# lauradarcy/gym-craftingworld

Measured on AMD Instinct MI355X. Metric: env-steps/sec at 65536 envs, 1/2/4/8 MI355X; bit-exact vs CPU ref, higher is better.
Workload: dtype u8

## Files before the change

### gym_craftingworld_amd/csrc/cw_kernels.hip

```cpp
#include <hip/hip_runtime.h>
#include <stdint.h>

#include "cw_host.h"
#include "cw_layout.h"
#include "cw_mt.h"

#define CW_WAVE 64
#define CW_BALLOT(p) __builtin_amdgcn_ballot_w64(p)
#define CW_ALT_FRAME_PACE 2

#ifdef CW_TRACE
__device__ unsigned long long cw_trace_buf[1024 * 8];
#define CW_STAMP(env, k) do { if (lane == 0) { cw_trace_buf[((env) & 1023) * 8 + (k)] = wall_clock64(); \
                                               if ((k) == 0 || (k) == 5) cw_trace_buf[((env) & 1023) * 8 + 6 + ((k) ? 1 : 0)] = clock64(); } } while (0)
extern "C" hipError_t cwk_trace_read(unsigned long long *dst) { return hipMemcpyFromSymbol(dst, HIP_SYMBOL(cw_trace_buf), sizeof(cw_trace_buf)); }
#else
#define CW_STAMP(env, k) do { } while (0)
#endif

enum { EMPTY = 0, STICKS = 1, AXE = 2, HAMMER = 3, ROCK = 4, TREE = 5, BREAD = 6, HOUSE = 7, WHEAT = 8 };
enum { T_MAKEBREAD = 0, T_EATBREAD = 1, T_BUILDHOUSE = 2, T_CHOPTREE = 3, T_CHOPROCK = 4,
       T_GOTOHOUSE = 5, T_MOVEAXE = 6, T_MOVEHAMMER = 7, T_MOVESTICKS = 8 };

typedef uint32_t u32x3 __attribute__((ext_vector_type(3)));
typedef u32x3 u32x3_a4 __attribute__((aligned(4)));

__device__ __forceinline__ void unpack_pos(const uint4 &v, uint32_t sp[8])
{
    sp[0] = v.x & 0xFFFFu; sp[1] = v.x >> 16;
    sp[2] = v.y & 0xFFFFu; sp[3] = v.y >> 16;
    sp[4] = v.z & 0xFFFFu; sp[5] = v.z >> 16;
    sp[6] = v.w & 0xFFFFu; sp[7] = v.w >> 16;
}
__device__ __forceinline__ uint4 pack_pos(const uint32_t sp[8])
{
    return make_uint4(sp[0] | (sp[1] << 16), sp[2] | (sp[3] << 16), sp[4] | (sp[5] << 16), sp[6] | (sp[7] << 16));
}
__device__ __forceinline__ int slot_at(const uint32_t sp[8], uint32_t cell)
{
    int idx = -1;
#pragma unroll
    for (int k = 0; k < 8; k++) idx = (sp[k] == cell) ? k : idx;
    return idx;
}
__device__ __forceinline__ uint32_t code_of(uint32_t codes, int idx)
{
    return idx < 0 ? 0u : ((codes >> (4 * idx)) & 15u);
}
__device__ __forceinline__ uint32_t rgb_of_code(uint32_t code)
{
    uint32_t c = 0;
    c = code == 1 ? (110u | (69u << 8) | (39u << 16)) : c;
    c = code == 2 ? (255u | (105u << 8) | (180u << 16)) : c;
    c = code == 3 ? (100u | (100u << 8) | (200u << 16)) : c;
    c = code == 4 ? (100u | (100u << 8) | (100u << 16)) : c;
    c = code == 5 ? (0u | (128u << 8) | (0u << 16)) : c;
    c = code == 6 ? (205u | (133u << 8) | (63u << 16)) : c;
    c = code == 7 ? (197u | (91u << 8) | (97u << 16)) : c;
    c = code == 8 ? (240u | (230u << 8) | (140u << 16)) : c;
    return c;
}

__device__ __forceinline__ u32x3 cell_row_dwords(uint32_t rgb)
{
    u32x3 d;
    d.x = rgb | (rgb << 24);
    d.y = (rgb >> 8) | (rgb << 16);
    d.z = (rgb >> 16) | (rgb << 8);
    return d;
}
__device__ __forceinline__ u32x3 overlay_dwords(u32x3 d, uint32_t o)
{
    d.x = (d.x & 0x00FFFFFFu) | (o << 24);
    d.y = (o >> 8) | (o << 16);
    d.z = (d.z & 0xFFFFFF00u) | (o >> 16);
    return d;
}
__device__ __forceinline__ u32x3 onehot_dwords(uint32_t bits)
{
    u32x3 d;
    d.x = (bits & 1u) | ((bits >> 1 & 1u) << 8) | ((bits >> 2 & 1u) << 16) | ((bits >> 3 & 1u) << 24);
    d.y = (bits >> 4 & 1u) | ((bits >> 5 & 1u) << 8) | ((bits >> 6 & 1u) << 16) | ((bits >> 7 & 1u) << 24);
    d.z = (bits >> 8 & 1u) | ((bits >> 9 & 1u) << 8) | ((bits >> 10 & 1u) << 16) | ((bits >> 11 & 1u) << 24);
    return d;
}

__device__ __forceinline__ void paint_cell(uint8_t *frame, int S, uint32_t cell, uint32_t code,
                                           bool agent_here, uint32_t hold, uint32_t div_magic, bool mark_rows_only = false)
{
    const uint32_t r = __umulhi(cell, div_magic);
    const uint32_t c = cell - r * S;
    const uint32_t rgb = rgb_of_code(code);
    const u32x3 base = cell_row_dwords(rgb);
    const uint32_t row_bytes = 12u * S;
    uint8_t *p = frame + (size_t)(4u * r) * row_bytes + 12u * c;
#pragma unroll
    for (int dy = 0; dy < 4; dy++) {
        u32x3 d = base;
        if (agent_here && (dy == 1 || dy == 2)) {
            uint32_t o = (dy == 2 && hold != 0) ? rgb_of_code(hold) : 0x00FFFFFFu;
            d = overlay_dwords(d, o);
        }
        if (dy == 1 || dy == 2 || !mark_rows_only) *(u32x3_a4 *)(p + dy * row_bytes) = d;
    }
}

__device__ __forceinline__ uint32_t cpv_color(int k)
{
    return k == 0 ? (45u | (82u << 8) | (160u << 16)) : k == 1 ? (255u | (102u << 8) | (102u << 16))
         : k == 2 ? (204u | (204u << 8)) : k == 3 ? (211u | (211u << 8) | (211u << 16))
         : k == 4 ? (34u | (133u << 8) | (34u << 16)) : k == 5 ? ((215u << 8) | (255u << 16))
         : k == 6 ? (153u | (52u << 8) | (255u << 16)) : k == 7 ? (10u | (215u << 8) | (100u << 16)) : (255u << 16);
}
__device__ __forceinline__ void alt_paint_tile(uint8_t *frame, int S, uint32_t r, uint32_t c, uint32_t code,
                                               bool agent_here, uint32_t hold)
{
    const uint32_t row_bytes = 9u * S;
    uint8_t *p = frame + (size_t)(3u * r) * row_bytes + 9u * c;
#pragma unroll
    for (int k = 0; k < 9; k++) {
        uint32_t cnt = (k < 8) ? (code == (uint32_t)(k + 1) ? 1u : 0u) : (agent_here ? 1u : 0u);
        if (k < 3) cnt += (agent_here && hold == (uint32_t)(k + 1)) ? 1u : 0u;
        const uint32_t col = cpv_color(k);
        uint8_t *q = p + (k / 3) * row_bytes + (k % 3) * 3;
        q[0] = (uint8_t)(cnt * (col & 0xFFu));
        q[1] = (uint8_t)(cnt * ((col >> 8) & 0xFFu));
        q[2] = (uint8_t)(cnt * ((col >> 16) & 0xFFu));
    }
}
__device__ __forceinline__ void alt_paint_strip(uint8_t *frame, int S, uint32_t hold, uint32_t first, uint32_t step,
                                                bool whole)
// ... 55 lines not shown
            for (int z = 0; z < pace; z++) __builtin_amdgcn_s_sleep(1);
        }
        if (p_any) {
            dst[p_off] = (uint8_t)p_val;
            dst[p_off + 1] = (uint8_t)(p_val >> 8);
            dst[p_off + 2] = (uint8_t)(p_val >> 16);
        }
    }
}

__device__ __forceinline__ void render_frame(uint8_t *__restrict__ dst0, uint8_t *__restrict__ dst1,
                                             int S, int ncell, uint32_t div_magic, const uint32_t sp[8],
                                             const uint32_t rgb[8], uint32_t agent_cell, uint32_t hold_rgb,
                                             int lane)
{
    const uint32_t row_bytes = 12u * S;
    for (uint32_t cell = lane; cell < (uint32_t)ncell; cell += CW_WAVE) {
        const uint32_t r = __umulhi(cell, div_magic);
        const uint32_t c = cell - r * S;
        uint32_t col = 0;
#pragma unroll
        for (int k = 0; k < 8; k++) col = (cell == sp[k]) ? rgb[k] : col;
        const u32x3 d = cell_row_dwords(col);
        const bool ag = (cell == agent_cell);
        const u32x3 d1 = ag ? overlay_dwords(d, 0x00FFFFFFu) : d;
        const u32x3 d2 = ag ? overlay_dwords(d, hold_rgb) : d;
        const size_t off = (size_t)(4u * r) * row_bytes + 12u * c;
        uint8_t *q = dst0 + off;
        *(u32x3_a4 *)(q) = d;
        *(u32x3_a4 *)(q + row_bytes) = d1;
        *(u32x3_a4 *)(q + 2 * row_bytes) = d2;
        *(u32x3_a4 *)(q + 3 * row_bytes) = d;
        if (dst1) {
            uint8_t *q1 = dst1 + off;
            *(u32x3_a4 *)(q1) = d;
            *(u32x3_a4 *)(q1 + row_bytes) = d1;
            *(u32x3_a4 *)(q1 + 2 * row_bytes) = d2;
            *(u32x3_a4 *)(q1 + 3 * row_bytes) = d;
        }
    }
}
template <bool kRecords = false>
__device__ __forceinline__ void paint_state_frame(const CwParams &P, uint8_t *dst, const uint32_t sp[8], uint32_t codes, uint32_t agent_cell,
                                                  uint32_t hold, int lane, uint8_t *dst1 = nullptr)
{
    if (P.raster == 1) {
        render_frame_alt<kRecords>(dst, dst1, P.size, P.ncell, P.div_magic, sp, codes, agent_cell, hold, lane, CW_ALT_FRAME_PACE);
    } else {
        uint32_t rgb[8];
#pragma unroll
        for (int k = 0; k < 8; k++) rgb[k] = rgb_of_code((codes >> (4 * k)) & 15u);
        render_frame(dst, dst1, P.size, P.ncell, P.div_magic, sp, rgb, agent_cell, hold ? rgb_of_code(hold) : 0x00FFFFFFu, lane);
    }
}
__device__ __forceinline__ uint32_t agent_cell_of(const CwParams &P, uint32_t hx) { return (hx & 0xFFu) * P.size + ((hx >> 8) & 0xFFu); }
__device__ __forceinline__ uint32_t hold_of(uint32_t hx) { return (hx >> 16) & 0xFFu; }
enum { CW_SRC_CURRENT = 0, CW_SRC_INIT = 1, CW_SRC_GOAL = 2 };
__device__ __forceinline__ void load_state_uniform(const CwParams &P, int env, int src, uint32_t sp[8], uint32_t &codes, uint32_t &agent_cell, uint32_t &hold)
{
    uint4 v_p;
    uint32_t v_c, v_a, v_h = 0;
    if (src == CW_SRC_CURRENT) {
        const uint4 h = P.hdr[env];
        v_p = P.pos[env];
        v_c = h.w;
        v_a = agent_cell_of(P, h.x);
        v_h = hold_of(h.x);
    } else if (src == CW_SRC_INIT) {
        v_p = P.init_pos[env];
        v_c = CW_CODES_INITIAL;
        v_a = P.init_agent[env];
    } else {
        v_p = P.goal_pos[env];
        v_c = P.goal_codes[env];
        v_a = P.goal_agent[env];
    }
    unpack_pos(make_uint4(__builtin_amdgcn_readfirstlane(v_p.x), __builtin_amdgcn_readfirstlane(v_p.y), __builtin_amdgcn_readfirstlane(v_p.z),
                          __builtin_amdgcn_readfirstlane(v_p.w)), sp);
    codes = __builtin_amdgcn_readfirstlane(v_c);
    agent_cell = __builtin_amdgcn_readfirstlane(v_a);
    hold = __builtin_amdgcn_readfirstlane(v_h);
}

struct CwStepOut {
    int reward;
    bool done, success, invalid, changed;
    uint32_t dirty0, dirty1;
    bool mark0, mark1;
    uint32_t step_num, achieved, desired;
    uint32_t n_success;
};

__device__ __forceinline__ int32_t episode_return_of(const CwParams &P, const CwStepOut &o)
{
    return (int32_t)o.n_success * (P.max_steps + 1) - (int32_t)o.step_num;
}

template <typename InitPosFn>
__device__ __forceinline__ CwStepOut step_env(const CwParams &P, uint4 &h, uint32_t sp[8], int a, InitPosFn load_init_pos)
{
    CwStepOut o;
    const int S = P.size;
    int ar = h.x & 0xFF, ac = (h.x >> 8) & 0xFF;
    uint32_t hold = (h.x >> 16) & 0xFF;
    uint32_t achieved = h.y & 0xFFFFu;
    const uint32_t desired = h.y >> 16;
    const uint32_t step_num = min((h.z & 0xFFFFu) + 1u, 0xFFFFu);
    const uint32_t flags = (h.z >> 16) & ~CW_FLAG_RESET;
    uint32_t codes = h.w;

    o.invalid = (unsigned)a > 5u;
    bool changed = false;
    const uint32_t cell = ar * S + ac;
    const int idx_here = slot_at(sp, cell);
    const uint32_t code_here = code_of(codes, idx_here);
    o.dirty0 = cell;
    o.dirty1 = 0xFFFFFFFFu;
    o.mark0 = o.mark1 = false;

    if (a == 4) {
        if (code_here >= STICKS && code_here <= HAMMER && hold == 0) {
            hold = code_here;
#pragma unroll
            for (int k = 0; k < 8; k++) sp[k] = (k == idx_here) ? CW_POS_HELD : sp[k];
            changed = true;
        }
    } else if (a == 5) {
        if (hold != 0 && idx_here < 0) {
#pragma unroll
            for (int k = 0; k < 8; k++) sp[k] = (sp[k] == CW_POS_HELD) ? cell : sp[k];
            hold = 0;
            changed = true;
        }
    } else if (!o.invalid) {
        const int dr = (a == 0) ? -1 : (a == 2) ? 1 : 0;
        const int dc = (a == 1) ? 1 : (a == 3) ? -1 : 0;
        const int nr = min(max(ar + dr, 0), S - 1);
        const int nc = min(max(ac + dc, 0), S - 1);
        uint32_t old_obj = 0;
        uint32_t cur_code = code_here;
        if (nr != ar || nc != ac) {
            const uint32_t ncell = nr * S + nc;
            const int idx_t = slot_at(sp, ncell);
            const uint32_t t = code_of(codes, idx_t);
            const bool cant = (t == ROCK && hold != 3) || (t == TREE && hold != 2);
            if (!cant) {
                changed = true;
                o.dirty1 = ncell;
                o.mark0 = true;
                ar = nr; ac = nc;
                old_obj = t;
                uint32_t nw = t;
                if (t == ROCK || t == BREAD) nw = EMPTY;
                else if (t == TREE) nw = STICKS;
                else if (t == STICKS && hold == 3) nw = HOUSE;
                else if (t == WHEAT && hold == 2) nw = BREAD;
                if (nw != t) {
                    codes = (codes & ~(15u << (4 * idx_t))) | (nw << (4 * idx_t));
                    if (nw == EMPTY) {
#pragma unroll
                        for (int k = 0; k < 8; k++) sp[k] = (k == idx_t) ? CW_POS_GONE : sp[k];
                    }
                }
                cur_code = nw;
                o.mark1 = nw == t;
            }
        }
        const uint32_t pcell = ar * S + ac;
        if (old_obj == BREAD) achieved |= 1u << T_EATBREAD;
        else if (old_obj == ROCK) achieved |= 1u << T_CHOPROCK;
        else if (old_obj == TREE) achieved |= 1u << T_CHOPTREE;
        achieved = (cur_code == HOUSE) ? (achieved | (1u << T_GOTOHOUSE))
                                       : (achieved & ~(1u << T_GOTOHOUSE));
        if (hold != 0) {
            const uint4 ip = load_init_pos();
            const uint32_t ip_sticks = ip.x & 0xFFFFu, ip_axe = ip.x >> 16;
            const uint32_t ip_hammer = ip.y & 0xFFFFu, ip_tree = ip.z & 0xFFFFu;
            if (hold == 1) {
                const bool home = (pcell == ip_sticks) ||
                                  (pcell == ip_tree && (achieved & (1u << T_CHOPTREE)));
                achieved = home ? (achieved & ~(1u << T_MOVESTICKS)) : (achieved | (1u << T_MOVESTICKS));
            } else if (hold == 2) {
                if (old_obj == WHEAT) achieved |= 1u << T_MAKEBREAD;
                achieved = (pcell == ip_axe) ? (achieved & ~(1u << T_MOVEAXE)) : (achieved | (1u << T_MOVEAXE));
            } else {
                if (old_obj == STICKS) achieved |= 1u << T_BUILDHOUSE;
                achieved = (pcell == ip_hammer) ? (achieved & ~(1u << T_MOVEHAMMER)) : (achieved | (1u << T_MOVEHAMMER));
            }
        }
    }

    int reward = -1;
    if (changed) {
        const uint32_t am = achieved & P.task_mask, dm = desired & P.task_mask;
        bool hit;
        if (flags & CW_FLAG_SUBSET)
            hit = ((dm & ~am) == 0) && (((~(dm ^ am)) & P.task_mask) != 0);
        else
            hit = (am == dm);
        reward = hit ? P.max_steps : -1;
    }
    o.reward = reward;
    o.changed = changed;
    o.success = (reward == P.max_steps);
    o.done = (step_num >= (uint32_t)P.max_steps) || o.success;
    o.step_num = step_num;
    o.achieved = achieved;
    o.desired = desired;
    o.n_success = min((flags >> 2) + (o.success ? 1u : 0u), 0x3FFFu);

    h.x = (uint32_t)ar | ((uint32_t)ac << 8) | (hold << 16) | (h.x & 0xFF000000u);
    h.y = achieved | (desired << 16);
    h.z = step_num | (((flags & 3u) | (o.n_success << 2)) << 16);
    h.w = codes;
    return o;
}

__device__ __forceinline__ void paint_changed_cells(const CwParams &P, int env, const uint4 &h, const uint32_t sp[8], const CwStepOut &o)
{
    uint8_t *frame = P.obs + (size_t)env * P.frame_bytes;
    const uint32_t hold = hold_of(h.x);
    const uint32_t acell = agent_cell_of(P, h.x);
    if (P.raster == 1) {
        const uint32_t r0 = __umulhi(o.dirty0, P.div_magic);
        alt_paint_tile(frame, P.size, r0, o.dirty0 - r0 * P.size, code_of(h.w, slot_at(sp, o.dirty0)), o.dirty0 == acell, hold);
        if (o.dirty1 != 0xFFFFFFFFu) {
            const uint32_t r1 = __umulhi(o.dirty1, P.div_magic);
            alt_paint_tile(frame, P.size, r1, o.dirty1 - r1 * P.size, code_of(h.w, slot_at(sp, o.dirty1)), o.dirty1 == acell, hold);
        }
        alt_paint_strip(frame, P.size, hold, 0, 1, false);
    } else {
        paint_cell(frame, P.size, o.dirty0, code_of(h.w, slot_at(sp, o.dirty0)), o.dirty0 == acell, hold, P.div_magic, o.mark0);
        if (o.dirty1 != 0xFFFFFFFFu)
            paint_cell(frame, P.size, o.dirty1, code_of(h.w, slot_at(sp, o.dirty1)), o.dirty1 == acell, hold, P.div_magic, o.mark1);
    }
}

__device__ __forceinline__ void store_step_outputs(const CwParams &P, int env, const CwStepOut &o)
{
    P.reward[env] = o.reward;
    P.done[env] = o.done ? 1 : 0;
    P.achieved_out[env] = (uint16_t)o.achieved;
    P.desired_out[env] = (uint16_t)o.desired;
    if (o.done) { P.episode_length[env] = (int32_t)o.step_num; P.episode_return[env] = episode_return_of(P, o); }
}

__device__ __forceinline__ int load_action(const void *actions, int act_dtype, int i)
{
    if (act_dtype == 0) return ((const int32_t *)actions)[i];
    if (act_dtype == 1) { const long long a = ((const long long *)actions)[i]; return a == (long long)(int)a ? (int)a : -1; }
    return ((const uint8_t *)actions)[i];
}

struct CwGoalState { uint4 pos; uint32_t codes, agent; };
__device__ __forceinline__ bool pop_next_episode(const CwParams &P, int env, uint32_t ctl, uint4 &h, uint32_t sp[8], bool count_episode, CwGoalState *goal = nullptr)
{
    const uint32_t slot = ctl & 0xFFu;
    const size_t at = (size_t)slot * P.n_envs + env;
    const uint4 m = P.nx_misc[at];
    const uint4 ipos = P.nx_init_pos[at];
    const uint4 gpos = P.nx_goal_pos[at];
    const int32_t ep_no = count_episode ? P.ep_no[env] : 0;
    if (!(m.z >> 31)) return false;
    P.init_pos[env] = ipos;
    P.goal_pos[env] = gpos;
    if (goal) { goal->pos = gpos; goal->codes = m.y; goal->agent = m.x >> 16; }
    P.goal_codes[env] = m.y;
    P.init_agent[env] = (uint16_t)(m.x & 0xFFFFu);
    P.goal_agent[env] = (uint16_t)(m.x >> 16);
    if (count_episode) P.ep_no[env] = ep_no + 1;
    ((uint32_t *)(P.nx_misc + at))[2] = 0;
    P.nx_ctl[env] = (slot + 1u == CW_LA_DEPTH ? 0u : slot + 1u) | CW_CTL_QUEUED;
    const uint32_t ia = m.x & 0xFFFFu;
    const uint32_t ar = __umulhi(ia, P.div_magic), ac = ia - ar * P.size;
    h.x = ar | (ac << 8) | (h.x & 0xFF000000u);
    h.y = (m.z & 0xFFFFu) << 16;
    h.z = (CW_FLAG_RESET | (((m.z >> 16) & 1u) ? CW_FLAG_SUBSET : 0u)) << 16;
    h.w = CW_CODES_INITIAL;
    unpack_pos(ipos, sp);
    return true;
}

__device__ __forceinline__ void note_slow_reset(const CwParams &P, int env, uint32_t ctl)
{
    atomicAdd(&P.counters[5], 1ull);
    if (!(ctl & CW_CTL_QUEUED)) P.nx_ctl[env] = ctl | CW_CTL_QUEUED;
}

__global__ __launch_bounds__(256) void cw_step_kernel(CwParams P, const void *actions, int act_dtype, int paint_dirty)
{
    const int i = blockIdx.x * blockDim.x + threadIdx.x;
    if (i == 0) {
        atomicAdd(&P.counters[0], (unsigned long long)P.n_envs);
    }
    const bool live = i < P.n_envs;
    bool done = false, success = false, invalid = false;
    if (live) {
        const int a = load_action(actions, act_dtype, i);
        uint4 h = P.hdr[i];
        uint32_t sp[8];
        unpack_pos(P.pos[i], sp);
        const CwStepOut o = step_env(P, h, sp, a, [&]() { return P.init_pos[i]; });
        done = o.done; success = o.success; invalid = o.invalid;

        P.hdr[i] = h;
        P.pos[i] = pack_pos(sp);
        store_step_outputs(P, i, o);
        if (paint_dirty && o.changed) paint_changed_cells(P, i, h, sp, o);
    }
    const unsigned long long m_done = CW_BALLOT(done), m_succ = CW_BALLOT(success), m_inv = CW_BALLOT(invalid);
    if ((m_done | m_inv) && (threadIdx.x & (CW_WAVE - 1)) == 0) {
        if (m_done) atomicAdd(&P.counters[1], (unsigned long long)__popcll(m_done));
        if (m_succ) atomicAdd(&P.counters[2], (unsigned long long)__popcll(m_succ));
        if (m_inv) atomicAdd(&P.counters[3], (unsigned long long)__popcll(m_inv));
    }
}

template <int A>
__device__ __forceinline__ void expand_one(const CwParams &P, const uint4 *__restrict__ hdr_in, const uint4 *__restrict__ pos_in, int j, int env, size_t row,
                                           const CwExpandOut &O)
{
    uint4 h = hdr_in[j];
    uint32_t sp[8];
    unpack_pos(pos_in[j], sp);
    const CwStepOut o = step_env(P, h, sp, A, [&]() { return P.init_pos[env]; });
    if (O.reward) O.reward[row] = o.reward;
    if (O.done) O.done[row] = o.done ? 1 : 0;
    if (O.changed) O.changed[row] = o.changed ? 1 : 0;
    if (O.achieved) O.achieved[row] = (uint16_t)o.achieved;
    if (O.hdr) O.hdr[row] = h;
    if (O.pos) O.pos[row] = pack_pos(sp);
}

__global__ __launch_bounds__(256) void cw_expand_kernel(CwParams P, const int32_t *__restrict__ env_of, const uint4 *__restrict__ hdr_in,
                                                        const uint4 *__restrict__ pos_in, int n_states, CwExpandOut O)
{
    const int j = (int)(blockIdx.x * blockDim.x + threadIdx.x);
    const int a = (int)blockIdx.y;
    int env = -1;
    bool skipped = false;
    if (j < n_states) {
        if (env_of) {
            const int32_t v = env_of[j];
            if (cwh_expand_env_ok(v, P.n_envs)) env = v;
            else skipped = v >= 0;
        } else {
            env = j < P.n_envs ? j : (int)((uint32_t)j % (uint32_t)P.n_envs);
        }
    }
    if (a == 0) {
        const unsigned long long m_skip = CW_BALLOT(skipped);
        if (m_skip && (threadIdx.x & (CW_WAVE - 1)) == 0) atomicAdd(&P.counters[7], (unsigned long long)__popcll(m_skip));
    }
    if (env < 0) return;
    const size_t row = (size_t)a * (size_t)n_states + (size_t)j;
    switch (a) {
    case 0: expand_one<0>(P, hdr_in, pos_in, j, env, row, O); break;
    case 1: expand_one<1>(P, hdr_in, pos_in, j, env, row, O); break;
    case 2: expand_one<2>(P, hdr_in, pos_in, j, env, row, O); break;
    case 3: expand_one<3>(P, hdr_in, pos_in, j, env, row, O); break;
    case 4: expand_one<4>(P, hdr_in, pos_in, j, env, row, O); break;
    case 5: expand_one<5>(P, hdr_in, pos_in, j, env, row, O); break;
    default: break;
    }
}

#define CW_SIM_BLOCK 8
__global__ __launch_bounds__(256) void cw_simulate_kernel(CwParams P, const int32_t *__restrict__ env_of, const uint4 *__restrict__ hdr_in,
                                                          const uint4 *__restrict__ pos_in, int own, int n_states, const uint8_t *__restrict__ actions,
                                                          int T, int stop_at_done, CwSimulateOut O)
{
    const int j = (int)(blockIdx.x * blockDim.x + threadIdx.x);
    int env = -1;
    bool skipped = false;
    if (j < n_states) {
        if (env_of) {
            const int32_t v = env_of[j];
            if (cwh_expand_env_ok(v, P.n_envs)) env = v;
            else skipped = v >= 0;
        } else {
            env = j < P.n_envs ? j : (int)((uint32_t)j % (uint32_t)P.n_envs);
        }
    }
    const unsigned long long m_skip = CW_BALLOT(skipped);
    if (m_skip && (threadIdx.x & (CW_WAVE - 1)) == 0) atomicAdd(&P.counters[7], (unsigned long long)__popcll(m_skip));
    if (env < 0) return;
    const size_t M = (size_t)n_states;
    const int src = own ? env : j;
    uint4 h = hdr_in[src];
    uint32_t sp[8];
    unpack_pos(pos_in[src], sp);
    const uint4 ip = P.init_pos[env];
    const uint8_t *const ap = actions + j;
    uint32_t raw[CW_SIM_BLOCK];
#pragma unroll
    for (int k = 0; k < CW_SIM_BLOCK; k++) raw[k] = ap[(size_t)min(k, T - 1) * M];
    int32_t ret = 0, length = T;
    bool active = true, any_done = false;
    int t0 = 0;
    for (; t0 < T; t0 += CW_SIM_BLOCK) {
        const uint32_t lo = raw[0] | (raw[1] << 8) | (raw[2] << 16) | (raw[3] << 24), hi = raw[4] | (raw[5] << 8) | (raw[6] << 16) | (raw[7] << 24);
        if (t0 + CW_SIM_BLOCK < T) {
#pragma unroll
            for (int k = 0; k < CW_SIM_BLOCK; k++) raw[k] = ap[(size_t)min(t0 + CW_SIM_BLOCK + k, T - 1) * M];
        }
        if (stop_at_done && !CW_BALLOT(active)) break;
        const int n = min(CW_SIM_BLOCK, T - t0);
        for (int k = 0; k < n; k++) {
// ... 560 lines not shown
    const int lane = threadIdx.x & (CW_WAVE - 1);
    const int wave_in_block = __builtin_amdgcn_readfirstlane(threadIdx.x / CW_WAVE);
    const CwBank E = engine_as_bank(P);
    for (int base = (int)blockIdx.x * epb; base < P.n_envs; base += (int)gridDim.x * epb) {
        const int mine = base + lane;
        const bool in_chunk = lane < epb && mine < P.n_envs;
        const int32_t v_row = in_chunk ? rows[mine] : -1;
        const bool v_in = cwh_snapshot_row_ok(v_row, B.rows) != 0;
        uint32_t v_valid = 0u;
        if (v_in) v_valid = B.valid[v_row];
        const bool v_ok = v_valid != 0u;
        unsigned long long m = CW_BALLOT(v_ok);
        const unsigned long long skipped = CW_BALLOT(v_row >= 0 && !v_ok);
        if (skipped && wave_in_block == 0 && lane == 0) atomicAdd(&P.counters[6], (unsigned long long)__builtin_popcountll(skipped));
        for (int rank = 0; m; rank++) {
            const int l = __builtin_ctzll(m);
            m &= m - 1;
            if ((rank & (CW_RESET_WAVES - 1)) != wave_in_block) continue;
            const int env = base + l;
            const size_t row = (size_t)__builtin_amdgcn_readlane(v_row, l);
            uint4 h = B.hdr[row];
            const uint4 ps = B.pos[row], ip = B.init_pos[row], gp = B.goal_pos[row];
            const uint32_t gc = B.goal_codes[row];
            const int32_t ep = B.ep_no[row];
            const uint32_t ia = B.init_agent[row], ga = B.goal_agent[row];
            if (with_stream) copy_stream_group(P, E, (size_t)env, B, row, lane);
            else h.x = (h.x & 0x00FFFFFFu) | (P.hdr[env].x & 0xFF000000u);
            if (lane == 0) {
                P.hdr[env] = h; P.pos[env] = ps; P.init_pos[env] = ip; P.goal_pos[env] = gp;
                P.goal_codes[env] = gc; P.ep_no[env] = ep; P.init_agent[env] = (uint16_t)ia; P.goal_agent[env] = (uint16_t)ga;
                P.achieved_out[env] = (uint16_t)(h.y & 0xFFFFu);
                P.desired_out[env] = (uint16_t)(h.y >> 16);
            }
            if constexpr (PAINT) {
                const size_t off = (size_t)env * P.frame_bytes;
                const uint32_t hx = __builtin_amdgcn_readfirstlane(h.x);
                uint32_t jp[8];
                unpack_pos(make_uint4(__builtin_amdgcn_readfirstlane(ps.x), __builtin_amdgcn_readfirstlane(ps.y), __builtin_amdgcn_readfirstlane(ps.z),
                                      __builtin_amdgcn_readfirstlane(ps.w)), jp);
                paint_state_frame(P, P.obs + off, jp, __builtin_amdgcn_readfirstlane(h.w), agent_cell_of(P, hx), hold_of(hx), lane);
                unpack_pos(make_uint4(__builtin_amdgcn_readfirstlane(ip.x), __builtin_amdgcn_readfirstlane(ip.y), __builtin_amdgcn_readfirstlane(ip.z),
                                      __builtin_amdgcn_readfirstlane(ip.w)), jp);
                paint_state_frame(P, P.init_img + off, jp, CW_CODES_INITIAL, __builtin_amdgcn_readfirstlane(ia), 0u, lane);
                unpack_pos(make_uint4(__builtin_amdgcn_readfirstlane(gp.x), __builtin_amdgcn_readfirstlane(gp.y), __builtin_amdgcn_readfirstlane(gp.z),
                                      __builtin_amdgcn_readfirstlane(gp.w)), jp);
                paint_state_frame(P, P.desired_img + off, jp, __builtin_amdgcn_readfirstlane(gc), __builtin_amdgcn_readfirstlane(ga), 0u, lane);
            }
        }
    }
}

__global__ __launch_bounds__(CW_RESET_WAVES *CW_WAVE) void cw_refill_kernel(CwParams P, int all_envs)
{
    __shared__ uint32_t s_mt[CW_RESET_WAVES][CW_MT_WORDS];
    const int lane = threadIdx.x & (CW_WAVE - 1);
    const int wave_in_block = __builtin_amdgcn_readfirstlane(threadIdx.x / CW_WAVE);
    const int wave = blockIdx.x * CW_RESET_WAVES + wave_in_block;
    const int n_waves = gridDim.x * CW_RESET_WAVES;
    if (P.la_feedback && blockIdx.x == 0 && threadIdx.x == 0)
        __hip_atomic_store(P.la_feedback, P.counters[5], __ATOMIC_RELAXED, __HIP_MEMORY_SCOPE_SYSTEM);
    enum { CHUNK = 16 };
    for (int base = wave * CHUNK; base < P.n_envs; base += n_waves * CHUNK) {
        const int mine = base + lane;
        const uint32_t v_ctl = (lane < CHUNK && mine < P.n_envs) ? P.nx_ctl[mine] : 0u;
        unsigned long long m = CW_BALLOT(lane < CHUNK && mine < P.n_envs && (all_envs || (v_ctl & CW_CTL_QUEUED)));
        while (m) {
            const int l = __builtin_ctzll(m);
            m &= m - 1;
            const int env = base + l;
            const uint32_t ctl = __builtin_amdgcn_readlane(v_ctl, l);
            const uint32_t v_hx = P.hdr[env].x;
            const uint32_t head = ctl & 0xFFu;
            for (uint32_t k = 0; k < CW_LA_DEPTH; k++) {
                const uint32_t slot = head + k >= CW_LA_DEPTH ? head + k - CW_LA_DEPTH : head + k;
                if (__builtin_amdgcn_readfirstlane(P.nx_misc[(size_t)slot * P.n_envs + env].z) >> 31) continue;
                const CwResetOut r = reset_env_wave(P, env, [&]() { return __builtin_amdgcn_readfirstlane(v_hx) >> 24; }, s_mt[wave_in_block], lane);
                if (lane == 0) store_next_record(P, env, (int)slot, r);
            }
            if ((ctl & CW_CTL_QUEUED) && lane == 0) P.nx_ctl[env] = head;
        }
    }
}

__global__ __launch_bounds__(CW_RESET_WAVES *CW_WAVE) void cw_rollout_kernel(CwParams P, const uint8_t *actions, int T,
                                                                             int32_t *rewards, uint8_t *dones, int epw)
{
    __shared__ uint32_t s_mt[CW_RESET_WAVES][CW_MT_WORDS];
    const int lane = threadIdx.x & (CW_WAVE - 1);
    const int wave_in_block = __builtin_amdgcn_readfirstlane(threadIdx.x / CW_WAVE);
    const int wave = blockIdx.x * CW_RESET_WAVES + wave_in_block;
    const int env0 = wave * epw;
    if (env0 >= P.n_envs) return;
    const int env = env0 + lane;
    const bool live = lane < epw && env < P.n_envs;
    const int e = live ? env : env0;
    uint4 h = P.hdr[e];
    uint32_t sp[8];
    unpack_pos(P.pos[e], sp);
    uint4 ip = P.init_pos[e];
    uint32_t ctl = P.lookahead ? P.nx_ctl[e] : 0u;
    unsigned long long n_done = 0, n_succ = 0, n_inv = 0;
    int reward = -1;
    bool done = false;
    uint32_t achieved = 0, desired = 0, step_num = 0;
    for (int t = 0; t < T; t++) {
        const int a = actions[(size_t)t * P.n_envs + e];
        const CwStepOut o = step_env(P, h, sp, a, [&]() { return ip; });
        reward = o.reward; done = o.done; achieved = o.achieved; desired = o.desired; step_num = o.step_num;
        if (live) {
            if (rewards) rewards[(size_t)t * P.n_envs + env] = o.reward;
            if (dones) dones[(size_t)t * P.n_envs + env] = o.done ? 1 : 0;
        }
        const unsigned long long m_all = CW_BALLOT(live && o.done);
        n_done += __popcll(m_all);
        n_succ += __popcll(CW_BALLOT(live && o.success));
        n_inv += __popcll(CW_BALLOT(live && o.invalid));
        if (m_all && live && o.done) { P.episode_length[env] = (int32_t)o.step_num; P.episode_return[env] = episode_return_of(P, o); }
        bool popped = false;
        const uint32_t ctl_was = ctl;
        if (live && o.done && P.lookahead) {
            popped = pop_next_episode(P, env, ctl, h, sp, true);
            if (popped) { ip = pack_pos(sp); ctl = ((ctl & 0xFFu) + 1u == CW_LA_DEPTH ? 0u : (ctl & 0xFFu) + 1u) | CW_CTL_QUEUED; }
        }
        const unsigned long long m_pop = CW_BALLOT(popped);
        unsigned long long m = m_all & ~m_pop;
        while (m) {
            const int l = __builtin_ctzll(m);
            m &= m - 1;
            const int env_l = env0 + l;
            const uint32_t menu_id = __builtin_amdgcn_readlane(h.x, l) >> 24;
            const CwResetOut r = reset_env_wave(P, env_l, [&]() { return menu_id; }, s_mt[wave_in_block], lane);
            if (lane == 0) {
                store_episode_records(P, env_l, r, true);
                if (P.lookahead) note_slow_reset(P, env_l, __builtin_amdgcn_readlane(ctl_was, l));
            }
            if (lane == l) {
                h = reset_header(P, r, menu_id);
                unpack_pos(r.init_pos, sp);
                ip = r.init_pos;
                ctl |= CW_CTL_QUEUED;
            }
        }
    }
    if (live) {
        P.hdr[env] = h;
        P.pos[env] = pack_pos(sp);
        P.reward[env] = reward;
        P.done[env] = done ? 1 : 0;
        P.achieved_out[env] = (uint16_t)achieved;
        P.desired_out[env] = (uint16_t)desired;
        (void)step_num;
    }
    if (lane == 0) {
        atomicAdd(&P.counters[0], (unsigned long long)min(epw, P.n_envs - env0) * (unsigned long long)T);
        if (n_done) atomicAdd(&P.counters[1], n_done);
        if (n_succ) atomicAdd(&P.counters[2], n_succ);
        if (n_inv) atomicAdd(&P.counters[3], n_inv);
    }
}

__global__ __launch_bounds__(CW_WAVE) void cw_resident_kernel(CwParams P, CwResident *R, uint32_t seq0, int paint_dirty,
                                                              unsigned long long idle_ticks, unsigned long long life_ticks)
{
    const int lane = threadIdx.x;
    uint4 h = P.hdr[0];
    uint32_t sp[8];
    unpack_pos(P.pos[0], sp);
    const uint4 ip = P.init_pos[0];
    uint32_t last = seq0;
    const unsigned long long t_start = wall_clock64();
    unsigned long long t_last = t_start;
    uint32_t reason = 0;
    for (;;) {
        const unsigned long long bell = __hip_atomic_load(&R->bell, __ATOMIC_ACQUIRE, __HIP_MEMORY_SCOPE_SYSTEM);
        const uint32_t d = (uint32_t)bell;
        const uint32_t seq = d >> 8;
        if (seq != last) {
            if (lane == 0) {
                const int a = (int)(d & 0x7Fu);
                const CwStepOut o = step_env(P, h, sp, a, [&]() { return ip; });
                P.hdr[0] = h;
                P.pos[0] = pack_pos(sp);
                store_step_outputs(P, 0, o);
                if (paint_dirty && o.changed) paint_changed_cells(P, 0, h, sp, o);
                atomicAdd(&P.counters[0], 1ull);
                if (o.done) atomicAdd(&P.counters[1], 1ull);
                if (o.success) atomicAdd(&P.counters[2], 1ull);
                if (o.invalid) atomicAdd(&P.counters[3], 1ull);
            }
            if (P.res_onehot && (d & 0x80u)) {
                const uint32_t hx = __builtin_amdgcn_readlane(h.x, 0), codes = __builtin_amdgcn_readlane(h.w, 0);
                uint32_t bp[8];
#pragma unroll
                for (int k = 0; k < 8; k++) bp[k] = __builtin_amdgcn_readlane(sp[k], 0);
                const uint32_t agent_cell = agent_cell_of(P, hx), hold = hold_of(hx);
                for (int cell = lane; cell < P.ncell; cell += CW_WAVE) {
                    const uint32_t code = code_of(codes, slot_at(bp, (uint32_t)cell));
                    uint32_t bits = code ? (1u << (code - 1)) : 0u;
                    if ((uint32_t)cell == agent_cell) bits |= (1u << 8) | (hold ? (1u << (8 + hold)) : 0u);
                    *(u32x3_a4 *)(P.res_onehot + 12 * cell) = onehot_dwords(bits);
                }
            }
            __threadfence_system();
            if (lane == 0) __hip_atomic_store(&R->ack, seq, __ATOMIC_RELEASE, __HIP_MEMORY_SCOPE_SYSTEM);
            last = seq;
            t_last = wall_clock64();
            continue;
        }
        const unsigned long long now = wall_clock64();
        if (bell >> 32) { reason = 1; break; }
        if (now - t_last > idle_ticks) { reason = 2; break; }
        if (now - t_start > life_ticks) { reason = 3; break; }
    }
    if (lane == 0) __hip_atomic_store(&R->exited, reason | (last << 8), __ATOMIC_RELEASE, __HIP_MEMORY_SCOPE_SYSTEM);
}

struct CwPaintJob { uint4 pos; uint32_t codes, agent_hold_kind, env, pad; };
enum { CW_JOB_INIT = 0, CW_JOB_GOAL = 1, CW_JOB_TERMINAL = 2 };
template <int PAINT, bool TERM>
__device__ __forceinline__ void fused_step(const CwParams &P, const void *actions, int act_dtype, int epw, int wave, uint32_t *s_mt_wave,
                                           CwPaintJob *s_jobs, int *s_njobs, int *s_cnt )
{
    constexpr int paint = PAINT;
    const int lane = threadIdx.x & (CW_WAVE - 1);
    const int wave_in_block = __builtin_amdgcn_readfirstlane(threadIdx.x / CW_WAVE);
    const int env0 = wave * epw;
    const bool wave_live = env0 < P.n_envs;
    const int env = env0 + lane;
    const bool live = wave_live && lane < epw && env < P.n_envs;
    const int e = live ? env : (wave_live ? env0 : 0);
    const int a = load_action(actions, act_dtype, e);
    uint4 h = P.hdr[e];
    uint32_t sp[8];
    unpack_pos(P.pos[e], sp);
    const uint4 ip = P.init_pos[e];
// ... 921 lines not shown
```

Baseline: 317.5 million.

## Rewrite step_env branch-free and replace per-step wave ballots with end-of-rollout reduction

Moves step_env into a shared host/device header and rewrites it as branchless predicated code: both slot lookups are done up front, the init-pos load is hoisted, and sp/codes/achieved are updated through selects. The goal is to remove divergent branches across the 64-lane wave, since each lane takes a different action. The rollout kernel also replaces three ballot+popcount operations per step with per-lane counters reduced once by shuffles at the end, and uses strided row pointers instead of recomputing indices. The price is extra ALU work per step, because every path is now always evaluated, and the bit-exact semantics have to hold across all the rewritten conditionals.

```diff
diff --git a/gym_craftingworld_amd/csrc/cw_kernels.hip b/gym_craftingworld_amd/csrc/cw_kernels.hip
--- a/gym_craftingworld_amd/csrc/cw_kernels.hip
+++ b/gym_craftingworld_amd/csrc/cw_kernels.hip
@@ -4,6 +4,7 @@
 #include "cw_host.h"
 #include "cw_layout.h"
 #include "cw_mt.h"
+#include "cw_step_env.h"
 
 #define CW_WAVE 64
 #define CW_BALLOT(p) __builtin_amdgcn_ballot_w64(p)
@@ -18,35 +19,9 @@
 #define CW_STAMP(env, k) do { } while (0)
 #endif
 
-enum { EMPTY = 0, STICKS = 1, AXE = 2, HAMMER = 3, ROCK = 4, TREE = 5, BREAD = 6, HOUSE = 7, WHEAT = 8 };
-enum { T_MAKEBREAD = 0, T_EATBREAD = 1, T_BUILDHOUSE = 2, T_CHOPTREE = 3, T_CHOPROCK = 4,
-       T_GOTOHOUSE = 5, T_MOVEAXE = 6, T_MOVEHAMMER = 7, T_MOVESTICKS = 8 };
-
 typedef uint32_t u32x3 __attribute__((ext_vector_type(3)));
 typedef u32x3 u32x3_a4 __attribute__((aligned(4)));
 
-__device__ __forceinline__ void unpack_pos(const uint4 &v, uint32_t sp[8])
-{
-    sp[0] = v.x & 0xFFFFu; sp[1] = v.x >> 16;
-    sp[2] = v.y & 0xFFFFu; sp[3] = v.y >> 16;
-    sp[4] = v.z & 0xFFFFu; sp[5] = v.z >> 16;
-    sp[6] = v.w & 0xFFFFu; sp[7] = v.w >> 16;
-}
-__device__ __forceinline__ uint4 pack_pos(const uint32_t sp[8])
-{
-    return make_uint4(sp[0] | (sp[1] << 16), sp[2] | (sp[3] << 16), sp[4] | (sp[5] << 16), sp[6] | (sp[7] << 16));
-}
-__device__ __forceinline__ int slot_at(const uint32_t sp[8], uint32_t cell)
-{
-    int idx = -1;
-#pragma unroll
-    for (int k = 0; k < 8; k++) idx = (sp[k] == cell) ? k : idx;
-    return idx;
-}
-__device__ __forceinline__ uint32_t code_of(uint32_t codes, int idx)
-{
-    return idx < 0 ? 0u : ((codes >> (4 * idx)) & 15u);
-}
 __device__ __forceinline__ uint32_t rgb_of_code(uint32_t code)
 {
     uint32_t c = 0;
@@ -268,139 +243,6 @@
     hold = __builtin_amdgcn_readfirstlane(v_h);
 }
 
-struct CwStepOut {
-    int reward;
-    bool done, success, invalid, changed;
-    uint32_t dirty0, dirty1;
-    bool mark0, mark1;
-    uint32_t step_num, achieved, desired;
-    uint32_t n_success;
-};
-
-__device__ __forceinline__ int32_t episode_return_of(const CwParams &P, const CwStepOut &o)
-{
-    return (int32_t)o.n_success * (P.max_steps + 1) - (int32_t)o.step_num;
-}
-
-template <typename InitPosFn>
-__device__ __forceinline__ CwStepOut step_env(const CwParams &P, uint4 &h, uint32_t sp[8], int a, InitPosFn load_init_pos)
-{
-    CwStepOut o;
-    const int S = P.size;
-    int ar = h.x & 0xFF, ac = (h.x >> 8) & 0xFF;
-    uint32_t hold = (h.x >> 16) & 0xFF;
-    uint32_t achieved = h.y & 0xFFFFu;
-    const uint32_t desired = h.y >> 16;
-    const uint32_t step_num = min((h.z & 0xFFFFu) + 1u, 0xFFFFu);
-    const uint32_t flags = (h.z >> 16) & ~CW_FLAG_RESET;
-    uint32_t codes = h.w;
-
-    o.invalid = (unsigned)a > 5u;
-    bool changed = false;
-    const uint32_t cell = ar * S + ac;
-    const int idx_here = slot_at(sp, cell);
-    const uint32_t code_here = code_of(codes, idx_here);
-    o.dirty0 = cell;
-    o.dirty1 = 0xFFFFFFFFu;
-    o.mark0 = o.mark1 = false;
-
-    if (a == 4) {
-        if (code_here >= STICKS && code_here <= HAMMER && hold == 0) {
-            hold = code_here;
-#pragma unroll
-            for (int k = 0; k < 8; k++) sp[k] = (k == idx_here) ? CW_POS_HELD : sp[k];
-            changed = true;
-        }
-    } else if (a == 5) {
-        if (hold != 0 && idx_here < 0) {
-#pragma unroll
-            for (int k = 0; k < 8; k++) sp[k] = (sp[k] == CW_POS_HELD) ? cell : sp[k];
-            hold = 0;
-            changed = true;
-        }
-    } else if (!o.invalid) {
-        const int dr = (a == 0) ? -1 : (a == 2) ? 1 : 0;
-        const int dc = (a == 1) ? 1 : (a == 3) ? -1 : 0;
-        const int nr = min(max(ar + dr, 0), S - 1);
-        const int nc = min(max(ac + dc, 0), S - 1);
-        uint32_t old_obj = 0;
-        uint32_t cur_code = code_here;
-        if (nr != ar || nc != ac) {
-            const uint32_t ncell = nr * S + nc;
-            const int idx_t = slot_at(sp, ncell);
-            const uint32_t t = code_of(codes, idx_t);
-            const bool cant = (t == ROCK && hold != 3) || (t == TREE && hold != 2);
-            if (!cant) {
-                changed = true;
-                o.dirty1 = ncell;
-                o.mark0 = true;
-                ar = nr; ac = nc;
-                old_obj = t;
-                uint32_t nw = t;
-                if (t == ROCK || t == BREAD) nw = EMPTY;
-                else if (t == TREE) nw = STICKS;
-                else if (t == STICKS && hold == 3) nw = HOUSE;
-                else if (t == WHEAT && hold == 2) nw = BREAD;
-                if (nw != t) {
-                    codes = (codes & ~(15u << (4 * idx_t))) | (nw << (4 * idx_t));
-                    if (nw == EMPTY) {
-#pragma unroll
-                        for (int k = 0; k < 8; k++) sp[k] = (k == idx_t) ? CW_POS_GONE : sp[k];
-                    }
-                }
-                cur_code = nw;
-                o.mark1 = nw == t;
-            }
-        }
-        const uint32_t pcell = ar * S + ac;
-        if (old_obj == BREAD) achieved |= 1u << T_EATBREAD;
-        else if (old_obj == ROCK) achieved |= 1u << T_CHOPROCK;
-        else if (old_obj == TREE) achieved |= 1u << T_CHOPTREE;
-        achieved = (cur_code == HOUSE) ? (achieved | (1u << T_GOTOHOUSE))
-                                       : (achieved & ~(1u << T_GOTOHOUSE));
-        if (hold != 0) {
-            const uint4 ip = load_init_pos();
-            const uint32_t ip_sticks = ip.x & 0xFFFFu, ip_axe = ip.x >> 16;
-            const uint32_t ip_hammer = ip.y & 0xFFFFu, ip_tree = ip.z & 0xFFFFu;
-            if (hold == 1) {
-                const bool home = (pcell == ip_sticks) ||
-                                  (pcell == ip_tree && (achieved & (1u << T_CHOPTREE)));
-                achieved = home ? (achieved & ~(1u << T_MOVESTICKS)) : (achieved | (1u << T_MOVESTICKS));
-            } else if (hold == 2) {
-                if (old_obj == WHEAT) achieved |= 1u << T_MAKEBREAD;
-                achieved = (pcell == ip_axe) ? (achieved & ~(1u << T_MOVEAXE)) : (achieved | (1u << T_MOVEAXE));
-            } else {
-                if (old_obj == STICKS) achieved |= 1u << T_BUILDHOUSE;
-                achieved = (pcell == ip_hammer) ? (achieved & ~(1u << T_MOVEHAMMER)) : (achieved | (1u << T_MOVEHAMMER));
-            }
-        }
-    }
-
-    int reward = -1;
-    if (changed) {
-        const uint32_t am = achieved & P.task_mask, dm = desired & P.task_mask;
-        bool hit;
-        if (flags & CW_FLAG_SUBSET)
-            hit = ((dm & ~am) == 0) && (((~(dm ^ am)) & P.task_mask) != 0);
-        else
-            hit = (am == dm);
-        reward = hit ? P.max_steps : -1;
-    }
-    o.reward = reward;
-    o.changed = changed;
-    o.success = (reward == P.max_steps);
-    o.done = (step_num >= (uint32_t)P.max_steps) || o.success;
-    o.step_num = step_num;
-    o.achieved = achieved;
-    o.desired = desired;
-    o.n_success = min((flags >> 2) + (o.success ? 1u : 0u), 0x3FFFu);
-
-    h.x = (uint32_t)ar | ((uint32_t)ac << 8) | (hold << 16) | (h.x & 0xFF000000u);
-    h.y = achieved | (desired << 16);
-    h.z = step_num | (((flags & 3u) | (o.n_success << 2)) << 16);
-    h.w = codes;
-    return o;
-}
 
 __device__ __forceinline__ void paint_changed_cells(const CwParams &P, int env, const uint4 &h, const uint32_t sp[8], const CwStepOut &o)
 {
@@ -486,7 +328,8 @@
         uint4 h = P.hdr[i];
         uint32_t sp[8];
         unpack_pos(P.pos[i], sp);
-        const CwStepOut o = step_env(P, h, sp, a, [&]() { return P.init_pos[i]; });
+        const uint4 ip = P.init_pos[i];
+        const CwStepOut o = step_env(P, h, sp, a, [&]() { return ip; });
         done = o.done; success = o.success; invalid = o.invalid;
 
         P.hdr[i] = h;
@@ -509,7 +352,8 @@
     uint4 h = hdr_in[j];
     uint32_t sp[8];
     unpack_pos(pos_in[j], sp);
-    const CwStepOut o = step_env(P, h, sp, A, [&]() { return P.init_pos[env]; });
+    const uint4 ip = P.init_pos[env];
+    const CwStepOut o = step_env(P, h, sp, A, [&]() { return ip; });
     if (O.reward) O.reward[row] = o.reward;
     if (O.done) O.done[row] = o.done ? 1 : 0;
     if (O.changed) O.changed[row] = o.changed ? 1 : 0;
@@ -1236,6 +1080,14 @@
     }
 }
 
+__device__ __forceinline__ unsigned long long wave_sum(uint32_t v)
+{
+    unsigned long long s = v;
+#pragma unroll
+    for (int d = 1; d < CW_WAVE; d <<= 1) s += __shfl_xor(s, d, CW_WAVE);
+    return s;
+}
+
 __global__ __launch_bounds__(CW_RESET_WAVES *CW_WAVE) void cw_rollout_kernel(CwParams P, const uint8_t *actions, int T,
                                                                              int32_t *rewards, uint8_t *dones, int epw)
 {
@@ -1253,26 +1105,34 @@
     unpack_pos(P.pos[e], sp);
     uint4 ip = P.init_pos[e];
     uint32_t ctl = P.lookahead ? P.nx_ctl[e] : 0u;
-    unsigned long long n_done = 0, n_succ = 0, n_inv = 0;
+    const uint32_t le = (uint32_t)e;
+    const uint8_t *a_row = actions;
+    int32_t *r_row = rewards;
+    uint8_t *d_row = dones;
+    uint32_t c_done = 0, c_succ = 0, c_inv = 0;
     int reward = -1;
     bool done = false;
-    uint32_t achieved = 0, desired = 0, step_num = 0;
+    uint32_t achieved = 0, desired = 0;
     for (int t = 0; t < T; t++) {
-        const int a = actions[(size_t)t * P.n_envs + e];
+        const int a = a_row[le];
+        a_row += P.n_envs;
         const CwStepOut o = step_env(P, h, sp, a, [&]() { return ip; });
-        reward = o.reward; done = o.done; achieved = o.achieved; desired = o.desired; step_num = o.step_num;
+        reward = o.reward; done = o.done; achieved = o.achieved; desired = o.desired;
+        const bool fin = live & o.done;
         if (live) {
-            if (rewards) rewards[(size_t)t * P.n_envs + env] = o.reward;
-            if (dones) dones[(size_t)t * P.n_envs + env] = o.done ? 1 : 0;
-        }
-        const unsigned long long m_all = CW_BALLOT(live && o.done);
-        n_done += __popcll(m_all);
-        n_succ += __popcll(CW_BALLOT(live && o.success));
-        n_inv += __popcll(CW_BALLOT(live && o.invalid));
-        if (m_all && live && o.done) { P.episode_length[env] = (int32_t)o.step_num; P.episode_return[env] = episode_return_of(P, o); }
+            if (rewards) r_row[le] = o.reward;
+            if (dones) d_row[le] = o.done ? 1 : 0;
+        }
+        r_row += P.n_envs;
+        d_row += P.n_envs;
+        c_done += fin ? 1u : 0u;
+        c_succ += (live & o.success) ? 1u : 0u;
+        c_inv += (live & o.invalid) ? 1u : 0u;
+        const unsigned long long m_all = CW_BALLOT(fin);
+        if (fin) { P.episode_length[env] = (int32_t)o.step_num; P.episode_return[env] = episode_return_of(P, o); }
         bool popped = false;
         const uint32_t ctl_was = ctl;
-        if (live && o.done && P.lookahead) {
+        if (fin && P.lookahead) {
             popped = pop_next_episode(P, env, ctl, h, sp, true);
             if (popped) { ip = pack_pos(sp); ctl = ((ctl & 0xFFu) + 1u == CW_LA_DEPTH ? 0u : (ctl & 0xFFu) + 1u) | CW_CTL_QUEUED; }
         }
@@ -1303,8 +1163,8 @@
         P.done[env] = done ? 1 : 0;
         P.achieved_out[env] = (uint16_t)achieved;
         P.desired_out[env] = (uint16_t)desired;
-        (void)step_num;
-    }
+    }
+    const unsigned long long n_done = wave_sum(c_done), n_succ = wave_sum(c_succ), n_inv = wave_sum(c_inv);
     if (lane == 0) {
         atomicAdd(&P.counters[0], (unsigned long long)min(epw, P.n_envs - env0) * (unsigned long long)T);
         if (n_done) atomicAdd(&P.counters[1], n_done);
diff --git a/gym_craftingworld_amd/csrc/cw_step_env.h b/gym_craftingworld_amd/csrc/cw_step_env.h
--- /dev/null
+++ b/gym_craftingworld_amd/csrc/cw_step_env.h
@@ -0,0 +1,159 @@
+#pragma once
+#include <stdint.h>
+
+#if defined(__HIPCC__)
+#define CW_HD __host__ __device__ __forceinline__
+#define CW_UNROLL _Pragma("unroll")
+#else
+#define CW_HD static inline
+#define CW_UNROLL
+struct uint4 { uint32_t x, y, z, w; };
+static inline uint4 make_uint4(uint32_t x, uint32_t y, uint32_t z, uint32_t w) { uint4 v; v.x = x; v.y = y; v.z = z; v.w = w; return v; }
+#endif
+
+#include "cw_layout.h"
+
+enum { EMPTY = 0, STICKS = 1, AXE = 2, HAMMER = 3, ROCK = 4, TREE = 5, BREAD = 6, HOUSE = 7, WHEAT = 8 };
+enum { T_MAKEBREAD = 0, T_EATBREAD = 1, T_BUILDHOUSE = 2, T_CHOPTREE = 3, T_CHOPROCK = 4,
+       T_GOTOHOUSE = 5, T_MOVEAXE = 6, T_MOVEHAMMER = 7, T_MOVESTICKS = 8 };
+
+CW_HD void unpack_pos(const uint4 &v, uint32_t sp[8])
+{
+    sp[0] = v.x & 0xFFFFu; sp[1] = v.x >> 16;
+    sp[2] = v.y & 0xFFFFu; sp[3] = v.y >> 16;
+    sp[4] = v.z & 0xFFFFu; sp[5] = v.z >> 16;
+    sp[6] = v.w & 0xFFFFu; sp[7] = v.w >> 16;
+}
+CW_HD uint4 pack_pos(const uint32_t sp[8])
+{
+    return make_uint4(sp[0] | (sp[1] << 16), sp[2] | (sp[3] << 16), sp[4] | (sp[5] << 16), sp[6] | (sp[7] << 16));
+}
+CW_HD int slot_at(const uint32_t sp[8], uint32_t cell)
+{
+    int idx = -1;
+    CW_UNROLL
+    for (int k = 0; k < 8; k++) idx = (sp[k] == cell) ? k : idx;
+    return idx;
+}
+CW_HD uint32_t code_of(uint32_t codes, int idx)
+{
+    return idx < 0 ? 0u : ((codes >> (4 * idx)) & 15u);
+}
+#define CW_NO_SLOT 32u
+CW_HD uint32_t slot_shift_at(const uint32_t sp[8], uint32_t cell)
+{
+    uint32_t sh = CW_NO_SLOT;
+    CW_UNROLL
+    for (int k = 0; k < 8; k++) sh = (sp[k] == cell) ? (uint32_t)(4 * k) : sh;
+    return sh;
+}
+CW_HD uint32_t code_at_shift(uint32_t codes, uint32_t sh)
+{
+    return sh == CW_NO_SLOT ? 0u : ((codes >> (sh & 31u)) & 15u);
+}
+
+struct CwStepOut {
+    int reward;
+    bool done, success, invalid, changed;
+    uint32_t dirty0, dirty1;
+    bool mark0, mark1;
+    uint32_t step_num, achieved, desired;
+    uint32_t n_success;
+};
+
+CW_HD int32_t episode_return_of(const CwParams &P, const CwStepOut &o)
+{
+    return (int32_t)o.n_success * (P.max_steps + 1) - (int32_t)o.step_num;
+}
+
+template <typename InitPosFn>
+CW_HD CwStepOut step_env(const CwParams &P, uint4 &h, uint32_t sp[8], int a, InitPosFn load_init_pos)
+{
+    CwStepOut o;
+    const uint32_t S = (uint32_t)P.size & 0xFFFFu;
+    const uint32_t ar = h.x & 0xFFu, ac = (h.x >> 8) & 0xFFu;
+    const uint32_t hold = (h.x >> 16) & 0xFFu;
+    const uint32_t achieved = h.y & 0xFFFFu;
+    const uint32_t desired = h.y >> 16;
+    const uint32_t sn = (h.z & 0xFFFFu) + 1u;
+    const uint32_t step_num = sn < 0xFFFFu ? sn : 0xFFFFu;
+    const uint32_t flags = (h.z >> 16) & ~CW_FLAG_RESET;
+    const uint32_t codes = h.w;
+    const uint4 ip = load_init_pos();
+
+    const bool is_pick = a == 4, is_drop = a == 5, is_move = (unsigned)a < 4u;
+    const int dr = (a == 2 ? 1 : 0) - (a == 0 ? 1 : 0), dc = (a == 1 ? 1 : 0) - (a == 3 ? 1 : 0);
+    const int top = (int)S - 1;
+    int nr_i = (int)ar + dr, nc_i = (int)ac + dc;
+    nr_i = nr_i < 0 ? 0 : nr_i; nr_i = nr_i > top ? top : nr_i;
+    nc_i = nc_i < 0 ? 0 : nc_i; nc_i = nc_i > top ? top : nc_i;
+    const uint32_t nr = is_move ? (uint32_t)nr_i : ar, nc = is_move ? (uint32_t)nc_i : ac;
+    const uint32_t cell = ar * S + ac, tcell = nr * S + nc;
+
+    const uint32_t sh_here = slot_shift_at(sp, cell), sh_t = slot_shift_at(sp, tcell);
+    const uint32_t code_here = code_at_shift(codes, sh_here), t = code_at_shift(codes, sh_t);
+
+    const bool pick_ok = is_pick & (code_here >= STICKS) & (code_here <= HAMMER) & (hold == 0);
+    const bool drop_ok = is_drop & (hold != 0) & (sh_here == CW_NO_SLOT);
+    const bool cant = ((t == ROCK) & (hold != 3)) | ((t == TREE) & (hold != 2));
+    const bool move_ok = is_move & ((nr != ar) | (nc != ac)) & !cant;
+    const bool changed = pick_ok | drop_ok | move_ok;
+
+    uint32_t nw = t;
+    nw = ((t == ROCK) | (t == BREAD)) ? (uint32_t)EMPTY : nw;
+    nw = (t == TREE) ? (uint32_t)STICKS : nw;
+    nw = ((t == STICKS) & (hold == 3)) ? (uint32_t)HOUSE : nw;
+    nw = ((t == WHEAT) & (hold == 2)) ? (uint32_t)BREAD : nw;
+    const bool vanish = move_ok & ((t == ROCK) | (t == BREAD));
+    const uint32_t new_codes = move_ok ? codes ^ ((nw ^ t) << (sh_t & 31u)) : codes;
+
+    const uint32_t e_sh = pick_ok ? sh_here : vanish ? sh_t : CW_NO_SLOT;
+    const uint32_t e_val = drop_ok ? cell : pick_ok ? (uint32_t)CW_POS_HELD : (uint32_t)CW_POS_GONE;
+    CW_UNROLL
+    for (int k = 0; k < 8; k++) {
+        const bool hit = (drop_ok & (sp[k] == CW_POS_HELD)) | (e_sh == (uint32_t)(4 * k));
+        sp[k] = hit ? e_val : sp[k];
+    }
+    const uint32_t new_hold = pick_ok ? code_here : drop_ok ? 0u : hold;
+
+    const uint32_t old_obj = move_ok ? t : 0u;
+    const uint32_t cur_code = move_ok ? nw : code_here;
+    const uint32_t pcell = move_ok ? tcell : cell;
+    uint32_t ach = achieved;
+    ach |= (old_obj == BREAD ? 1u << T_EATBREAD : 0u) | (old_obj == ROCK ? 1u << T_CHOPROCK : 0u) | (old_obj == TREE ? 1u << T_CHOPTREE : 0u);
+    ach = (cur_code == HOUSE) ? (ach | (1u << T_GOTOHOUSE)) : (ach & ~(1u << T_GOTOHOUSE));
+    const uint32_t ip_sticks = ip.x & 0xFFFFu, ip_axe = ip.x >> 16, ip_hammer = ip.y & 0xFFFFu, ip_tree = ip.z & 0xFFFFu;
+    const uint32_t ip_tool = hold == 1 ? ip_sticks : hold == 2 ? ip_axe : ip_hammer;
+    const uint32_t tool_bit = hold == 0 ? 0u : hold == 1 ? 1u << T_MOVESTICKS : hold == 2 ? 1u << T_MOVEAXE : 1u << T_MOVEHAMMER;
+    const uint32_t craft = ((hold == 2) & (old_obj == WHEAT)) ? 1u << T_MAKEBREAD : ((hold > 2) & (old_obj == STICKS)) ? 1u << T_BUILDHOUSE : 0u;
+    const bool home = (pcell == ip_tool) | ((hold == 1) & (pcell == ip_tree) & ((ach & (1u << T_CHOPTREE)) != 0));
+    ach |= craft;
+    ach = home ? (ach & ~tool_bit) : (ach | tool_bit);
+    const uint32_t new_achieved = is_move ? ach : achieved;
+
+    const uint32_t am = new_achieved & P.task_mask, dm = desired & P.task_mask;
+    const bool hit_subset = ((dm & ~am) == 0) & (((~(dm ^ am)) & P.task_mask) != 0);
+    const bool hit_equal = am == dm;
+    const bool hit = (flags & CW_FLAG_SUBSET) ? hit_subset : hit_equal;
+    const int reward = (changed & hit) ? P.max_steps : -1;
+    o.reward = reward;
+    o.changed = changed;
+    o.invalid = (unsigned)a > 5u;
+    o.success = (reward == P.max_steps);
+    o.done = (step_num >= (uint32_t)P.max_steps) | o.success;
+    o.step_num = step_num;
+    o.achieved = new_achieved;
+    o.desired = desired;
+    const uint32_t ns = (flags >> 2) + (o.success ? 1u : 0u);
+    o.n_success = ns < 0x3FFFu ? ns : 0x3FFFu;
+    o.dirty0 = cell;
+    o.dirty1 = move_ok ? tcell : 0xFFFFFFFFu;
+    o.mark0 = move_ok;
+    o.mark1 = move_ok & (nw == t);
+
+    h.x = (move_ok ? nr | (nc << 8) : ar | (ac << 8)) | (new_hold << 16) | (h.x & 0xFF000000u);
+    h.y = new_achieved | (desired << 16);
+    h.z = step_num | (((flags & 3u) | (o.n_success << 2)) << 16);
+    h.w = new_codes;
+    return o;
+}
```

Result: no change. 315.5 million (-0.6%).
